# meta-pytorch/torchx

Measured on AMD Instinct MI355X. Metric: tokens_per_second, higher is better.
Workload: dtype bf16; 1 GPU; model=llama3_8b, global_batch=4, seq_len=4096, parallelism=dp1

## Files before the change

torchx_amd/models/llama.py:

```python

from __future__ import annotations

from dataclasses import dataclass
from typing import Optional

import torch
import torch.nn as nn

from torchx_amd import ops


@dataclass
class LlamaConfig:
    vocab_size: int = 128256
    hidden_size: int = 4096
    intermediate_size: int = 14336
    num_layers: int = 32
    num_heads: int = 32
    num_kv_heads: int = 8
    head_dim: int = 128
    max_seq_len: int = 8192
    rope_theta: float = 500000.0
    rms_eps: float = 1e-5
    tie_embeddings: bool = False

    @property
    def q_dim(self) -> int:
        return self.num_heads * self.head_dim

    @property
    def kv_dim(self) -> int:
        return self.num_kv_heads * self.head_dim


def llama3_8b() -> LlamaConfig:
    return LlamaConfig()

# ... 14 lines not shown
    )


def _lin(mod: nn.Module, x: torch.Tensor) -> torch.Tensor:
    if type(mod) is nn.Linear and mod.bias is None and x.is_cuda:
        return ops.fast_linear(x, mod.weight)
    return mod(x)


def _new_linear(in_features: int, out_features: int,
                device: Optional[torch.device]) -> nn.Linear:
    if device is not None and torch.device(device).type == "cuda":
        return torch.nn.utils.skip_init(
            nn.Linear, in_features, out_features, bias=False,
            dtype=torch.bfloat16, device=device)
    return nn.Linear(in_features, out_features, bias=False,
                     dtype=torch.bfloat16)


class LlamaBlock(nn.Module):
    def __init__(self, cfg: LlamaConfig,
                 device: Optional[torch.device] = None):
        super().__init__()
        self.cfg = cfg
        h, qd, kvd = cfg.hidden_size, cfg.q_dim, cfg.kv_dim
        self.wqkv = _new_linear(h, qd + 2 * kvd, device)
        self.wo = _new_linear(qd, h, device)
        self.wgu = _new_linear(h, 2 * cfg.intermediate_size, device)
        self.wdown = _new_linear(cfg.intermediate_size, h, device)
        self.attn_norm = nn.Parameter(torch.ones(h, dtype=torch.bfloat16))
        self.mlp_norm = nn.Parameter(torch.ones(h, dtype=torch.bfloat16))

    def forward(self, x: torch.Tensor, cos: torch.Tensor,
                sin: torch.Tensor) -> torch.Tensor:
        cfg = self.cfg
        B, S, H = x.shape
        xn = ops.rmsnorm(x, self.attn_norm, cfg.rms_eps)
        qkv = _lin(self.wqkv, xn)
        attn = ops.fused_attention_qkv(
            qkv, cos, sin, cfg.num_heads, cfg.num_kv_heads, causal=True
        )
        x = x + _lin(self.wo, attn.reshape(B, S, cfg.q_dim))
        xn = ops.rmsnorm(x, self.mlp_norm, cfg.rms_eps)
        x = x + _lin(self.wdown, ops.swiglu_packed(_lin(self.wgu, xn)))
        return x


class LlamaModel(nn.Module):

    def __init__(self, cfg: LlamaConfig, device: Optional[torch.device] = None):
        super().__init__()
        self.cfg = cfg
        factory = {"dtype": torch.bfloat16, "device": device}
        self.embed = nn.Embedding(cfg.vocab_size, cfg.hidden_size, **factory)
        self.blocks = nn.ModuleList(
            [LlamaBlock(cfg, device) for _ in range(cfg.num_layers)]
        )
        self.final_norm = nn.Parameter(
            torch.ones(cfg.hidden_size, dtype=torch.bfloat16)
        )
        self.lm_head = _new_linear(cfg.hidden_size, cfg.vocab_size, device)
        if cfg.tie_embeddings:
            self.lm_head.weight = self.embed.weight
        cos, sin = ops.rope_tables(cfg.max_seq_len, cfg.head_dim,
                                   cfg.rope_theta, device=device)
        self.register_buffer("rope_cos", cos, persistent=False)
        self.register_buffer("rope_sin", sin, persistent=False)
        if device is not None:
            self.to(device)
        self.apply(self._init_weights)

    def _init_weights(self, m: nn.Module) -> None:
        std = 0.02
        if isinstance(m, nn.Linear):
            nn.init.normal_(m.weight, mean=0.0, std=std)
        elif isinstance(m, nn.Embedding):
            nn.init.normal_(m.weight, mean=0.0, std=std)

    def forward_hidden(self, tokens: torch.Tensor) -> torch.Tensor:
        x = self.embed(tokens)
        cos, sin = self.rope_cos, self.rope_sin
        for blk in self.blocks:
            x = blk(x, cos, sin)
        return ops.rmsnorm(x, self.final_norm, self.cfg.rms_eps)

    def forward(self, tokens: torch.Tensor,
                targets: Optional[torch.Tensor] = None) -> torch.Tensor:
        x = self.forward_hidden(tokens)
        if targets is None:
            return self.lm_head(x)
        return ops.fused_linear_cross_entropy(
            x, self.lm_head.weight, targets
        )

    def num_params(self) -> int:
        return sum(p.numel() for p in self.parameters())
```

torchx_amd/ops/__init__.py:

```python

from __future__ import annotations

import importlib.util
import math
from pathlib import Path
from typing import Optional, Tuple

import torch

from . import reference

_SO = Path(__file__).resolve().parent / "_hip_ops.so"
_hip = None
_load_err: Optional[str] = None


def _load():
    global _hip, _load_err
    if _hip is not None:
        return _hip
    if not _SO.exists():
        _load_err = f"{_SO} not built (run torchx_amd/ops/build.py)"
        return None
    try:
# ... 15 lines not shown
            "back to eager."
        )
    return mod


def extension_available() -> bool:
    return _load() is not None


def _on_gpu(*ts: torch.Tensor) -> bool:
    return any(t.is_cuda for t in ts)




class _RMSNorm(torch.autograd.Function):
    @staticmethod
    def forward(ctx, x: torch.Tensor, w: torch.Tensor, eps: float):
        y, invrms = hip_ops().rmsnorm_fwd(x.contiguous(), w.contiguous(), eps)
        ctx.save_for_backward(x, w, invrms)
        return y

    @staticmethod
    def backward(ctx, dy: torch.Tensor):
        x, w, invrms = ctx.saved_tensors
        dx, dw = hip_ops().rmsnorm_bwd(dy.contiguous(), x, w, invrms)
        return dx, dw.to(w.dtype), None


def rmsnorm(x: torch.Tensor, w: torch.Tensor, eps: float = 1e-5) -> torch.Tensor:
    if _on_gpu(x):
        return _RMSNorm.apply(x, w, eps)
    return reference.rmsnorm(x, w, eps)




def rope_tables(
    seq_len: int, head_dim: int, theta: float = 500000.0,
    device: Optional[torch.device] = None,
) -> Tuple[torch.Tensor, torch.Tensor]:
    inv_freq = 1.0 / (
        theta ** (torch.arange(0, head_dim, 2, dtype=torch.float32) / head_dim)
    )
    pos = torch.arange(seq_len, dtype=torch.float32)
    ang = torch.outer(pos, inv_freq)
    cos, sin = torch.cos(ang), torch.sin(ang)
    if device is not None:
        cos, sin = cos.to(device), sin.to(device)
    return cos, sin


class _RoPE(torch.autograd.Function):
    @staticmethod
    def forward(ctx, x: torch.Tensor, cos: torch.Tensor, sin: torch.Tensor,
                heads: int):
        ctx.save_for_backward(cos, sin)
        ctx.heads = heads
        return hip_ops().rope(x.contiguous(), cos, sin, heads, 1.0)

    @staticmethod
    def backward(ctx, dy: torch.Tensor):
        cos, sin = ctx.saved_tensors
        dx = hip_ops().rope(dy.contiguous(), cos, sin, ctx.heads, -1.0)
        return dx, None, None, None

# ... 129 lines not shown
    def forward(ctx, q: torch.Tensor, k: torch.Tensor, v: torch.Tensor,
                causal: bool, scale: float):
        o, lse = hip_ops().attn_fwd(
            q.contiguous(), k.contiguous(), v.contiguous(), scale, causal
        )
        ctx.save_for_backward(q, k, v, o, lse)
        ctx.causal = causal
        ctx.scale = scale
        return o

    @staticmethod
    def backward(ctx, dout: torch.Tensor):
        q, k, v, o, lse = ctx.saved_tensors
        dq, dk, dv = hip_ops().attn_bwd(
            q, k, v, o, dout.contiguous(), lse, ctx.scale, ctx.causal
        )
        return dq, dk, dv, None, None


def set_attn_bwd_dq_mode(mode: str) -> None:
    hip_ops().set_attn_bwd_dq_mode(mode)


def get_attn_bwd_dq_mode() -> str:
    return hip_ops().get_attn_bwd_dq_mode()


def set_attn_bwd_dkv_impl(impl: str) -> None:
    hip_ops().set_attn_bwd_dkv_impl(impl)


def get_attn_bwd_dkv_impl() -> str:
    return hip_ops().get_attn_bwd_dkv_impl()


def flash_attention(
    q: torch.Tensor, k: torch.Tensor, v: torch.Tensor,
    causal: bool = True, scale: Optional[float] = None,
) -> torch.Tensor:
    if scale is None:
        scale = 1.0 / math.sqrt(q.shape[-1])
    if _on_gpu(q):
        return _FlashAttention.apply(q, k, v, causal, scale)
    return reference.attention(q, k, v, causal=causal, scale=scale)




def adamw_step(
    p32: torch.Tensor, p16: torch.Tensor, grad: torch.Tensor,
    m: torch.Tensor, v: torch.Tensor, *, lr: float, beta1: float = 0.9,
    beta2: float = 0.95, eps: float = 1e-8, weight_decay: float = 0.1,
    step: int = 1,
) -> None:
    if p32.is_cuda:
        hip_ops().adamw_step(p32, p16, grad, m, v, lr, beta1, beta2, eps,
                             weight_decay, step)
    else:
        reference.adamw_step(p32, p16, grad, m, v, lr=lr, beta1=beta1,
                             beta2=beta2, eps=eps, weight_decay=weight_decay,
                             step=step)


def mfma_probe(a: torch.Tensor, b: torch.Tensor) -> torch.Tensor:
    return hip_ops().mfma_probe(a, b)

# ... 347 lines not shown
```

torchx_amd/ops/csrc/attention.hip:

```cpp
#include "common.h"

#include <cstdlib>
#include <cstring>
#include <type_traits>

typedef __bf16 mbf16x8 __attribute__((ext_vector_type(8)));

#define HD 128
#define QBLK 32
#define KBLK 32
#define NWAVES 4
#define BLOCK_Q (QBLK * NWAVES)
#define BLOCK_K (KBLK * NWAVES)

__device__ __forceinline__ f32x16 mfma32(mbf16x8 a, mbf16x8 b, f32x16 c) {
  return __builtin_amdgcn_mfma_f32_32x32x16_bf16(a, b, c, 0, 0, 0);
}

__device__ __forceinline__ unsigned int pack_bf16x2(float a, float b) {
  unsigned int r;
  asm("v_cvt_pk_bf16_f32 %0, %1, %2" : "=v"(r) : "v"(a), "v"(b));
  return r;
}

// ... 115 lines not shown
  for (int p = 0; p < 4; ++p) {
    const int c = tid + p * 256;
    const int r = c >> 4, g = c & 15;
    #pragma unroll
    for (int j = 0; j < 8; ++j) {
      const int d = 8 * g + j;
      const int gr = ((r >> 3) + vrot(d)) & 7;
      *(unsigned short*)(vimg + d * 128 + gr * 16 + (r & 7) * 2) = vr[p][j];
    }
  }
}


__device__ __forceinline__ void map_block_fwd(int B, int Hq, int Hkv,
                                              int nqt, int G,
                                              int* b, int* hq, int* qt) {
  int bid = blockIdx.x;
  if (((B * Hkv) & 7) == 0) {
    const int gsz = G * nqt;
    const int xcd = bid & 7, slot = bid >> 3;
    const int g = (slot / gsz) * 8 + xcd;
    *b = g / Hkv;
    const int r = slot % gsz;
    *hq = (g % Hkv) * G + r / nqt;
    *qt = r % nqt;
  } else {
    *b = bid / (Hq * nqt);
    bid -= *b * Hq * nqt;
    *hq = bid / nqt;
    *qt = bid % nqt;
  }
}

template <int NTHREADS>
__device__ __forceinline__ void lds_nat_to_tr(const char* nat, char* tr_img) {
  const int tid = threadIdx.x;
  #pragma unroll
  for (int p = 0; p < 1024 / NTHREADS; ++p) {
    const int c = tid + p * NTHREADS;
    const int r = c >> 4, g = c & 15;
    const ushort8 v = *(const ushort8*)(
        nat + r * 256 + ((g * 16) ^ ((r & 15) << 4)));
    #pragma unroll
    for (int j = 0; j < 8; ++j) {
      const int d = 8 * g + j;
      const int gr = ((r >> 3) + vrot(d)) & 7;
      *(unsigned short*)(tr_img + d * 128 + gr * 16 + (r & 7) * 2) = v[j];
    }
  }
}



template <int NW = 4>
__device__ __forceinline__ void lds_nat_to_tr_own(const char* nat,
                                                  char* tr_img) {
  const int wave = threadIdx.x / 64;
  const int lane = threadIdx.x & 63;
  #pragma unroll
  for (int pp = 0; pp < 16 / NW; ++pp) {
    const int c = wave * (64 * 16 / NW) + pp * 64 + lane;
    const int r = c >> 4, g = c & 15;
    const ushort8 v = *(const ushort8*)(
        nat + r * 256 + ((g * 16) ^ ((r & 15) << 4)));
    #pragma unroll
    for (int j = 0; j < 8; ++j) {
      const int d = 8 * g + j;
      const int gr = ((r >> 3) + vrot(d)) & 7;
      *(unsigned short*)(tr_img + d * 128 + gr * 16 + (r & 7) * 2) = v[j];
    }
  }
}

template <int NW>
__global__ void __launch_bounds__(NW * 64, 2)
attn_fwd_kernel(const unsigned short* __restrict__ q,
                const unsigned short* __restrict__ k,
                const unsigned short* __restrict__ v,
                unsigned short* __restrict__ o,
                float* __restrict__ lse,
                int B, int S, int Hq, int Hkv, float scale, int causal,
                long q_rs, long kv_rs) {
  __shared__ __align__(16) char smem[4 * KIMG_BYTES];

  const int BQ = NW * QBLK;
  const int nqt = (S + BQ - 1) / BQ;
  const int G = Hq / Hkv;
  int b, hq, qt;
  map_block_fwd(B, Hq, Hkv, nqt, G, &b, &hq, &qt);
  const int hkv = hq / G;

  const int wave = threadIdx.x / 64;
  const int lane = threadIdx.x & 63;
  const bool hi = lane >= 32;
  const int qr = lane & 31;

  const long q_seq_stride = q_rs;
  const long kv_seq_stride = kv_rs;
  const unsigned short* qb = q + (long)b * S * q_seq_stride + (long)hq * HD;
  const unsigned short* kb = k + (long)b * S * kv_seq_stride + (long)hkv * HD;
  const unsigned short* vb = v + (long)b * S * kv_seq_stride + (long)hkv * HD;

  const int q0_blk = qt * BQ;
  const int qw0 = q0_blk + wave * QBLK;
  const long q_row = qw0 + qr;
  const bool wave_active = qw0 < S;

  mbf16x8 qfrag[8];
  {
    const long row = (q_row < S) ? q_row : (S - 1);
    const unsigned short* qp = qb + row * q_seq_stride + (hi ? 8 : 0);
    #pragma unroll
    for (int c = 0; c < 8; ++c) {
      qfrag[c] = __builtin_bit_cast(mbf16x8, *(const ushort8*)(qp + c * 16));
    }
  }

  f32x16 acc_o[4] = {};
  float m_run = -3.0e38f, l_run = 0.f;
  const float sc2 = scale * LOG2E;

  const int kv_limit = causal ? min(S, q0_blk + BQ) : S;
// ... 1318 lines not shown
    #pragma unroll
    for (int o = 0; o < 2; ++o) {
      unsigned short* out = o ? dk : dv;
      #pragma unroll
      for (int dt = 0; dt < 4; ++dt) {
        __syncthreads();
        #pragma unroll
        for (int r = 0; r < 16; ++r) {
          tr[c_row(r, hi) * 36 + kr] = o ? acck[dt][r] : accv[dt][r];
        }
        __syncthreads();
        #pragma unroll
        for (int rep = 0; rep < 4; ++rep) {
          const int kk = kr;
          const int d0 = (hi ? 16 : 0) + rep * 4;
          if (kw0 + kk < S) {
            bf16x4_raw w;
            #pragma unroll
            for (int j = 0; j < 4; ++j) {
              w[j] = (short)f32_to_bf16(tr[kk * 36 + d0 + j]);
            }
            *(bf16x4_raw*)(out + ((long)b * S + kw0 + kk) * out_rs +
                           (long)hkv * HD + dt * 32 + d0) = w;
          }
        }
      }
    }
  } else {
    #pragma unroll
    for (int i = 0; i < 16; ++i) __syncthreads();
  }
}

extern "C" void attn_fwd_launch(const void* q, const void* k, const void* v,
                                void* o, void* lse, int B, int S, int Hq,
                                int Hkv, float scale, int causal,
                                long q_rs, long kv_rs, hipStream_t stream) {
  static int fwd8 = -1;
  if (fwd8 < 0) {
    const char* e = getenv("TORCHX_AMD_FWD_8WAVE");
    fwd8 = (e && atoi(e)) ? 1 : 0;
  }
  if (fwd8 == 1) {
    const int nqt = (S + 8 * QBLK - 1) / (8 * QBLK);
    hipLaunchKernelGGL((attn_fwd_kernel<8>), dim3(B * Hq * nqt), dim3(512),
                       0, stream, (const unsigned short*)q,
                       (const unsigned short*)k, (const unsigned short*)v,
                       (unsigned short*)o, (float*)lse, B, S, Hq, Hkv,
                       scale, causal, q_rs, kv_rs);
  } else {
    const int nqt = (S + 4 * QBLK - 1) / (4 * QBLK);
    hipLaunchKernelGGL((attn_fwd_kernel<4>), dim3(B * Hq * nqt), dim3(256),
                       0, stream, (const unsigned short*)q,
                       (const unsigned short*)k, (const unsigned short*)v,
                       (unsigned short*)o, (float*)lse, B, S, Hq, Hkv,
                       scale, causal, q_rs, kv_rs);
  }
}

extern "C" void paged_prefill_attn_launch(
    const void* q, const void* kpool, const void* vpool, void* o,
    const void* bt, const void* ctx, int B, int S, int Hq, int Hkv,
    int num_pages, int logP, int M, float scale, hipStream_t stream) {
  const int nqt = (S + 4 * QBLK - 1) / (4 * QBLK);
  hipLaunchKernelGGL(paged_prefill_attn_kernel, dim3(B * Hq * nqt), dim3(256),
                     0, stream, (const unsigned short*)q,
                     (const unsigned short*)kpool,
                     (const unsigned short*)vpool, (unsigned short*)o,
                     (const int*)bt, (const int*)ctx, B, S, Hq, Hkv,
                     num_pages, logP, M, scale);
}

extern "C" void paged_prefill_attn_ragged_launch(
    const void* q, const void* kpool, const void* vpool, void* o,
    const void* bt, const void* ctx, const void* tiles, int ntiles, int B,
    int T, int Hq, int Hkv, int num_pages, int logP, int M, float scale,
    hipStream_t stream) {
  const long units = (long)ntiles * Hkv;
  const long grid = (units + 7) / 8 * 8 * (Hq / Hkv);
  hipLaunchKernelGGL(paged_prefill_attn_ragged_kernel, dim3((unsigned)grid),
                     dim3(256), 0, stream, (const unsigned short*)q,
                     (const unsigned short*)kpool,
                     (const unsigned short*)vpool, (unsigned short*)o,
                     (const int*)bt, (const int*)ctx, (const int4*)tiles,
                     ntiles, B, T, Hq, Hkv, num_pages, logP, M, scale);
}

static int g_dkv_merged = -1;

// ... 102 lines not shown
```

torchx_amd/ops/csrc/bindings.cpp:

```cpp
#include <torch/extension.h>
#include <c10/hip/HIPStream.h>

#include <hip/hip_runtime.h>

extern "C" {
void rope_launch(const void*, void*, const void*, const void*, long, int, int,
                 int, float, hipStream_t);
void swiglu_fwd_launch(const void*, const void*, void*, long, hipStream_t);
void swiglu_bwd_launch(const void*, const void*, const void*, void*, void*,
                       long, hipStream_t);
void rmsnorm_fwd_launch(const void*, const void*, void*, void*, long, int,
                        float, hipStream_t);
void rmsnorm_bwd_launch(const void*, const void*, const void*, const void*,
                        void*, void*, void*, long, int, hipStream_t);
long rmsnorm_bwd_dw_chunks(long);
void adamw_launch(void*, void*, const void*, void*, void*, long, float, float,
                  float, float, float, float, float, hipStream_t);
void ce_fwd_launch(const void*, const void*, void*, void*, long, int,
                   hipStream_t);
void ce_bwd_launch(const void*, const void*, const void*, const void*, void*,
                   long, int, hipStream_t);
void attn_fwd_launch(const void*, const void*, const void*, void*, void*, int,
                     int, int, int, float, int, long, long, hipStream_t);
void attn_bwd_launch(const void*, const void*, const void*, const void*,
                     const void*, const void*, void*, void*, void*, void*,
                     void*, int, int, int, int, float, int, long, long, long,
                     long, hipStream_t);
long attn_bwd_ds_bytes(int, int, int, int);
int attn_bwd_dkv_impl_get();
void attn_bwd_dkv_impl_set(int);
void rope_qkv_launch(const void*, void*, const void*, const void*, long, int,
                     long, int, float, hipStream_t);
void swiglu_gu_fwd_launch(const void*, void*, long, long, hipStream_t);
void swiglu_gu_bwd_launch(const void*, const void*, void*, long, long,
                          hipStream_t);
void mfma_probe_launch(const void*, const void*, void*, hipStream_t);
void mfma_probe_tr_launch(const void*, const void*, void*, void*,
                          hipStream_t);
void fp8_cast_transpose_launch(const void*, void*, void*, void*,
                               const void*, long, long, int, hipStream_t);
void transpose_bf16_launch(const void*, void*, long, long, hipStream_t);
void decode_attn_launch(const void*, const void*, const void*, void*,
                        const void*, int, int, int, int, int, int, float,
                        hipStream_t);
void gemv_bf16_launch(const void*, const void*, void*, int, int, int,
                      hipStream_t);
void decode_attn_split_launch(const void*, const void*, const void*, void*,
                              void*, void*, const void*, int, int, int, int,
                              int, int, int, float, hipStream_t);
void decode_rope_cache_launch(const void*, void*, void*, void*, const void*,
                              const void*, const void*, int, int, int, int,
                              int, int, hipStream_t);
void rmsnorm_res_launch(const void*, const void*, const void*, void*, void*,
                        long, int, float, hipStream_t);
void gemv_swiglu_launch(const void*, const void*, void*, int, int, int,
                        hipStream_t);
void paged_decode_attn_launch(const void*, const void*, const void*, void*,
                              void*, void*, const void*, const void*, int,
                              int, int, int, int, int, int, float,
                              hipStream_t);
void paged_decode_rope_cache_launch(const void*, void*, void*, void*,
                                    const void*, const void*, const void*,
                                    const void*, int, int, int, int, int,
                                    int, int, hipStream_t);
void paged_prefill_attn_launch(const void*, const void*, const void*, void*,
                               const void*, const void*, int, int, int, int,
                               int, int, int, float, hipStream_t);
void paged_prefill_attn_ragged_launch(const void*, const void*, const void*,
                                      void*, const void*, const void*,
                                      const void*, int, int, int, int, int,
                                      int, int, int, float, hipStream_t);
void paged_prefill_rope_cache_launch(const void*, void*, void*, void*,
                                     const void*, const void*, const void*,
                                     const void*, long, int, int, long, int,
                                     hipStream_t);
}

namespace {

hipStream_t cur_stream() {
  return c10::hip::getCurrentHIPStream().stream();
}

void check_bf16(const at::Tensor& t, const char* name) {
  TORCH_CHECK(t.is_cuda(), name, " must be on GPU");
  TORCH_CHECK(t.scalar_type() == at::kBFloat16, name, " must be bf16");
  TORCH_CHECK(t.is_contiguous(), name, " must be contiguous");
}

void check_f32(const at::Tensor& t, const char* name) {
  TORCH_CHECK(t.is_cuda(), name, " must be on GPU");
  TORCH_CHECK(t.scalar_type() == at::kFloat, name, " must be f32");
  TORCH_CHECK(t.is_contiguous(), name, " must be contiguous");
}

}

std::vector<at::Tensor> rmsnorm_fwd(at::Tensor x, at::Tensor w, double eps) {
  check_bf16(x, "x");
  check_bf16(w, "w");
  const long H = x.size(-1);
  TORCH_CHECK(H % 2048 == 0 && H <= 8192, "rmsnorm: H must be k*2048, <=8192");
  const long rows = x.numel() / H;
  auto y = at::empty_like(x);
  auto invrms = at::empty({rows}, x.options().dtype(at::kFloat));
  rmsnorm_fwd_launch(x.data_ptr(), w.data_ptr(), y.data_ptr(),
                     invrms.data_ptr(), rows, (int)H, (float)eps,
                     cur_stream());
  return {y, invrms};
}

std::vector<at::Tensor> rmsnorm_bwd(at::Tensor dy, at::Tensor x, at::Tensor w,
                                    at::Tensor invrms) {
  check_bf16(dy, "dy");
  check_bf16(x, "x");
  const long H = x.size(-1);
  TORCH_CHECK(H % 2048 == 0 && H <= 8192, "rmsnorm: H must be k*2048, <=8192");
  const long rows = x.numel() / H;
  auto dx = at::empty_like(x);
  auto dw = at::empty({H}, x.options().dtype(at::kFloat));
  auto dw_part = at::empty({rmsnorm_bwd_dw_chunks(rows), H}, dw.options());
  rmsnorm_bwd_launch(dy.data_ptr(), x.data_ptr(), w.data_ptr(),
                     invrms.data_ptr(), dx.data_ptr(), dw.data_ptr(),
                     dw_part.data_ptr(), rows, (int)H, cur_stream());
  return {dx, dw};
}

at::Tensor rope(at::Tensor x, at::Tensor cos_t, at::Tensor sin_t, long heads,
                double sign) {
  check_bf16(x, "x");
  check_f32(cos_t, "cos");
  check_f32(sin_t, "sin");
  const long D = x.size(-1);
  const long rows = x.numel() / D;
  const long S = cos_t.size(0);
  TORCH_CHECK(cos_t.size(1) == D / 2, "cos table must be [S, D/2]");
  auto y = at::empty_like(x);
  rope_launch(x.data_ptr(), y.data_ptr(), cos_t.data_ptr(), sin_t.data_ptr(),
              rows, (int)D, (int)heads, (int)S, (float)sign, cur_stream());
  return y;
}

at::Tensor swiglu_fwd(at::Tensor g, at::Tensor u) {
  check_bf16(g, "g");
  check_bf16(u, "u");
  auto out = at::empty_like(g);
  swiglu_fwd_launch(g.data_ptr(), u.data_ptr(), out.data_ptr(), g.numel(),
                    cur_stream());
  return out;
}

std::vector<at::Tensor> swiglu_bwd(at::Tensor dout, at::Tensor g,
                                   at::Tensor u) {
  check_bf16(dout, "dout");
  auto dg = at::empty_like(g);
  auto du = at::empty_like(u);
// ... 60 lines not shown
  return {o, lse};
}

int g_dq_stream = -1;

bool dq_stream_mode() {
  if (g_dq_stream < 0) {
    const char* e = getenv("TORCHX_AMD_DQ_MODE");
    g_dq_stream = (e && std::string(e) == "recompute") ? 0 : 1;
  }
  return g_dq_stream == 1;
}

void set_attn_bwd_dq_mode(const std::string& mode) {
  TORCH_CHECK(mode == "stream" || mode == "recompute",
              "attn bwd dq mode must be 'stream' or 'recompute', got '",
              mode, "'");
  g_dq_stream = (mode == "stream") ? 1 : 0;
}

std::string get_attn_bwd_dq_mode() {
  return dq_stream_mode() ? "stream" : "recompute";
}

void set_attn_bwd_dkv_impl(const std::string& impl) {
  TORCH_CHECK(impl == "merged" || impl == "split",
              "attn bwd dkv impl must be 'merged' or 'split', got '", impl,
              "'");
  attn_bwd_dkv_impl_set(impl == "merged" ? 1 : 0);
}

std::string get_attn_bwd_dkv_impl() {
  return attn_bwd_dkv_impl_get() == 1 ? "merged" : "split";
}

constexpr long kDsScratchCapBytes = 8L << 30;

at::Tensor alloc_ds_scratch(const at::Tensor& like, int B, int S, int Hq,
                            bool causal) {
  if (!dq_stream_mode()) return at::Tensor();
  const long bytes = attn_bwd_ds_bytes(B, S, Hq, causal ? 1 : 0);
  if (bytes > kDsScratchCapBytes) return at::Tensor();
  return at::empty({bytes}, like.options().dtype(at::kByte));
}

std::vector<at::Tensor> attn_bwd(at::Tensor q, at::Tensor k, at::Tensor v,
                                 at::Tensor o, at::Tensor dout, at::Tensor lse,
                                 double scale, bool causal) {
  check_bf16(dout, "dout");
  const int B = q.size(0), S = q.size(1), Hq = q.size(2);
  const int Hkv = k.size(2);
  auto dq = at::empty_like(q);
  auto dk = at::empty_like(k);
  auto dv = at::empty_like(v);
  auto delta = at::empty({B, Hq, S}, q.options().dtype(at::kFloat));
  auto ds = alloc_ds_scratch(q, B, S, Hq, causal);
  attn_bwd_launch(q.data_ptr(), k.data_ptr(), v.data_ptr(), o.data_ptr(),
                  dout.data_ptr(), lse.data_ptr(), delta.data_ptr(),
                  dq.data_ptr(), dk.data_ptr(), dv.data_ptr(),
                  ds.defined() ? ds.data_ptr() : nullptr, B, S, Hq, Hkv,
                  (float)scale, causal ? 1 : 0, (long)Hq * 128,
                  (long)Hkv * 128, (long)Hq * 128, (long)Hkv * 128,
                  cur_stream());
  return {dq, dk, dv};
}

// ... 394 lines not shown
              "cos/sin must be [S, 64] (head_dim 128)");
  const long nh = qkv.size(1) / 128;
  const int Hq = (int)nh - 2 * Hkv;
  TORCH_CHECK(Hq >= 1 && qkv.size(1) == nh * 128, "qkv width mismatch");
  TORCH_CHECK(Hq % Hkv == 0, "GQA group mismatch");
  const int rope_rows = (int)std::min<long>(cos_t.size(0), 1L << 30);
  auto q = at::empty({T, (long)Hq, 128}, qkv.options());
  paged_prefill_rope_cache_launch(
      qkv.data_ptr(), q.data_ptr(), kpool.data_ptr(), vpool.data_ptr(),
      cos_t.data_ptr(), sin_t.data_ptr(), pos.data_ptr(), slot.data_ptr(), T,
      Hq, Hkv, pool_rows, rope_rows, cur_stream());
  return q;
}

std::vector<at::Tensor> rmsnorm_res(at::Tensor x,
                                    c10::optional<at::Tensor> res,
                                    at::Tensor w, double eps) {
  check_bf16(x, "x");
  check_bf16(w, "w");
  const long H = x.size(-1);
  TORCH_CHECK(H % 2048 == 0 && H <= 8192, "rmsnorm: H must be k*2048, <=8192");
  const long R = x.numel() / H;
  auto y = at::empty_like(x);
  at::Tensor s = x;
  const void* rp = nullptr;
  void* sp = nullptr;
  if (res.has_value()) {
    check_bf16(*res, "res");
    TORCH_CHECK(res->sizes() == x.sizes(), "res shape mismatch");
    s = at::empty_like(x);
    rp = res->data_ptr();
    sp = s.data_ptr();
  }
  rmsnorm_res_launch(x.data_ptr(), rp, w.data_ptr(), sp, y.data_ptr(), R,
                     (int)H, (float)eps, cur_stream());
  return {s, y};
}

std::vector<at::Tensor> mfma_probe_tr(at::Tensor a, at::Tensor b) {
  check_bf16(a, "a");
  check_bf16(b, "b");
  TORCH_CHECK(a.size(0) == 32 && a.size(1) == 16, "a must be [32,16]");
  TORCH_CHECK(b.size(0) == 16 && b.size(1) == 32, "b must be [16,32]");
  auto c = at::empty({32, 32}, a.options().dtype(at::kFloat));
  auto raw = at::empty({64, 8}, a.options());
  mfma_probe_tr_launch(a.data_ptr(), b.data_ptr(), c.data_ptr(),
                       raw.data_ptr(), cur_stream());
  return {c, raw};
}

at::Tensor mfma_probe(at::Tensor a, at::Tensor b) {
  check_bf16(a, "a");
  check_bf16(b, "b");
  TORCH_CHECK(a.size(0) == 32 && a.size(1) == 16, "a must be [32,16]");
  TORCH_CHECK(b.size(0) == 16 && b.size(1) == 32, "b must be [16,32]");
  auto c = at::empty({32, 32}, a.options().dtype(at::kFloat));
  mfma_probe_launch(a.data_ptr(), b.data_ptr(), c.data_ptr(), cur_stream());
  return c;
}

PYBIND11_MODULE(TORCH_EXTENSION_NAME, m) {
  m.def("rmsnorm_fwd", &rmsnorm_fwd);
  m.def("rmsnorm_bwd", &rmsnorm_bwd);
  m.def("rope", &rope);
  m.def("swiglu_fwd", &swiglu_fwd);
  m.def("swiglu_bwd", &swiglu_bwd);
  m.def("adamw_step", &adamw_step);
  m.def("ce_fwd", &ce_fwd);
  m.def("ce_bwd", &ce_bwd);
  m.def("attn_fwd", &attn_fwd);
  m.def("attn_bwd", &attn_bwd);
  m.def("set_attn_bwd_dq_mode", &set_attn_bwd_dq_mode);
  m.def("get_attn_bwd_dq_mode", &get_attn_bwd_dq_mode);
  m.def("set_attn_bwd_dkv_impl", &set_attn_bwd_dkv_impl);
  m.def("get_attn_bwd_dkv_impl", &get_attn_bwd_dkv_impl);
  m.def("attn_fwd_qkv", &attn_fwd_qkv);
  m.def("attn_bwd_qkv", &attn_bwd_qkv);
  m.def("rope_qkv", &rope_qkv);
  m.def("swiglu_gu_fwd", &swiglu_gu_fwd);
  m.def("swiglu_gu_bwd", &swiglu_gu_bwd);
  m.def("fp8_cast_transpose", &fp8_cast_transpose);
  m.def("mfma_probe", &mfma_probe);
  m.def("mfma_probe_tr", &mfma_probe_tr);
  m.def("transpose_bf16", &transpose_bf16);
  m.def("decode_attn", &decode_attn);
  m.def("decode_attn_dev", &decode_attn_dev);
  m.def("gemv_bf16", &gemv_bf16);
  m.def("gemv_swiglu_bf16", &gemv_swiglu_bf16);
  m.def("decode_rope_cache", &decode_rope_cache,
        py::arg("qkv"), py::arg("kc"), py::arg("vc"), py::arg("cos"),
        py::arg("sin"), py::arg("pos") = 0,
        py::arg("pos_dev") = c10::nullopt);
  m.def("paged_decode_attn", &paged_decode_attn);
  m.def("paged_decode_rope_cache", &paged_decode_rope_cache);
  m.def("paged_prefill_attn", &paged_prefill_attn);
  m.def("paged_prefill_attn_ragged", &paged_prefill_attn_ragged);
  m.def("paged_prefill_rope_cache", &paged_prefill_rope_cache);
  m.def("rmsnorm_res", &rmsnorm_res,
        py::arg("x"), py::arg("res"), py::arg("w"), py::arg("eps"));
}
```

torchx_amd/ops/csrc/rmsnorm.hip:

```cpp
#include "common.h"

template <int ITERS>
__global__ void __launch_bounds__(256)
rmsnorm_fwd_kernel(
    const unsigned short* __restrict__ x,
    const unsigned short* __restrict__ w,
    unsigned short* __restrict__ y,
    float* __restrict__ invrms,
    int H, float eps) {
  __shared__ float red[4];
  const long row = blockIdx.x;
  const unsigned short* xr = x + row * (long)H;
  unsigned short* yr = y + row * (long)H;

  float xs[ITERS][8];
  float acc = 0.f;
  #pragma unroll
  for (int it = 0; it < ITERS; ++it) {
    int i = (it * 256 + threadIdx.x) * 8;
    ushort8 v = *(const ushort8*)(xr + i);
    #pragma unroll
    for (int j = 0; j < 8; ++j) {
      float f = bf16_to_f32(v[j]);
      xs[it][j] = f;
      acc = fmaf(f, f, acc);
    }
  }
  float total = block_reduce<4>(acc, red,
      [] __device__ (float a, float b) { return a + b; });
  float r = rsqrtf(total / (float)H + eps);
  if (threadIdx.x == 0) invrms[row] = r;

  #pragma unroll
  for (int it = 0; it < ITERS; ++it) {
    int i = (it * 256 + threadIdx.x) * 8;
    ushort8 wv = *(const ushort8*)(w + i);
    ushort8 ov;
    #pragma unroll
    for (int j = 0; j < 8; ++j) {
      ov[j] = f32_to_bf16(xs[it][j] * r * bf16_to_f32(wv[j]));
    }
    *(ushort8*)(yr + i) = ov;
  }
}


template <int ITERS>
__global__ void __launch_bounds__(256)
rmsnorm_bwd_dx_kernel(
    const unsigned short* __restrict__ dy,
    const unsigned short* __restrict__ x,
    const unsigned short* __restrict__ w,
    const float* __restrict__ invrms,
    unsigned short* __restrict__ dx,
    int H) {
  __shared__ float red[4];
  const long row = blockIdx.x;
  const unsigned short* xr = x + row * (long)H;
  const unsigned short* dyr = dy + row * (long)H;
  unsigned short* dxr = dx + row * (long)H;
  const float r = invrms[row];

  float xs[ITERS][8], dyw[ITERS][8];
  float t = 0.f;
  #pragma unroll
  for (int it = 0; it < ITERS; ++it) {
    int i = (it * 256 + threadIdx.x) * 8;
    ushort8 xv = *(const ushort8*)(xr + i);
    ushort8 dv = *(const ushort8*)(dyr + i);
    ushort8 wv = *(const ushort8*)(w + i);
    #pragma unroll
    for (int j = 0; j < 8; ++j) {
      float xf = bf16_to_f32(xv[j]);
      float dwf = bf16_to_f32(dv[j]) * bf16_to_f32(wv[j]);
      xs[it][j] = xf;
      dyw[it][j] = dwf;
      t = fmaf(dwf, xf, t);
    }
  }
  float ts = block_reduce<4>(t, red,
      [] __device__ (float a, float b) { return a + b; });
  const float kk = ts * r * r * r / (float)H;

  #pragma unroll
  for (int it = 0; it < ITERS; ++it) {
    int i = (it * 256 + threadIdx.x) * 8;
    ushort8 ov;
    #pragma unroll
    for (int j = 0; j < 8; ++j) {
      ov[j] = f32_to_bf16(fmaf(dyw[it][j], r, -xs[it][j] * kk));
    }
    *(ushort8*)(dxr + i) = ov;
  }
}

#define DW_CHUNK_ROWS 64

__global__ void __launch_bounds__(256)
rmsnorm_bwd_dw_kernel(
    const unsigned short* __restrict__ dy,
    const unsigned short* __restrict__ x,
    const float* __restrict__ invrms,
    float* __restrict__ part,
    long rows, int H) {
  const int col = (blockIdx.y * 2048) + threadIdx.x * 8;
  const long row0 = (long)blockIdx.x * DW_CHUNK_ROWS;
  const long row1 = min(row0 + DW_CHUNK_ROWS, rows);
  float acc[8] = {0.f, 0.f, 0.f, 0.f, 0.f, 0.f, 0.f, 0.f};
  for (long row = row0; row < row1; ++row) {
    const float r = invrms[row];
    ushort8 xv = *(const ushort8*)(x + row * (long)H + col);
    ushort8 dv = *(const ushort8*)(dy + row * (long)H + col);
    #pragma unroll
    for (int j = 0; j < 8; ++j) {
      acc[j] = fmaf(bf16_to_f32(dv[j]) * bf16_to_f32(xv[j]), r, acc[j]);
    }
  }
  float* out = part + (long)blockIdx.x * H + col;
  #pragma unroll
  for (int j = 0; j < 8; ++j) out[j] = acc[j];
}

__global__ void __launch_bounds__(256)
// ... 10 lines not shown
  red[group][lane] = s;
  __syncthreads();
  if (group == 0) {
    dw[col] = (red[0][lane] + red[1][lane]) + (red[2][lane] + red[3][lane]);
  }
}

extern "C" long rmsnorm_bwd_dw_chunks(long rows) {
  return (rows + DW_CHUNK_ROWS - 1) / DW_CHUNK_ROWS;
}

#define DISPATCH_ITERS(H, FN)                                                  \
  do {                                                                         \
    int iters = (H) / 2048;                                                    \
    if (iters == 1) FN(1);                                                     \
    else if (iters == 2) FN(2);                                                \
    else if (iters == 3) FN(3);                                                \
    else if (iters == 4) FN(4);                                                \
  } while (0)

extern "C" void rmsnorm_fwd_launch(const void* x, const void* w, void* y,
                                   void* invrms, long rows, int H, float eps,
                                   hipStream_t stream) {
#define LAUNCH_F(I)                                                            \
  hipLaunchKernelGGL((rmsnorm_fwd_kernel<I>), dim3((int)rows), dim3(256), 0,   \
                     stream, (const unsigned short*)x,                         \
                     (const unsigned short*)w, (unsigned short*)y,             \
                     (float*)invrms, H, eps)
  DISPATCH_ITERS(H, LAUNCH_F);
#undef LAUNCH_F
}

extern "C" void rmsnorm_bwd_launch(const void* dy, const void* x,
                                   const void* w, const void* invrms, void* dx,
                                   void* dw, void* dw_part, long rows, int H,
                                   hipStream_t stream) {
#define LAUNCH_B(I)                                                            \
  hipLaunchKernelGGL((rmsnorm_bwd_dx_kernel<I>), dim3((int)rows), dim3(256),   \
                     0, stream, (const unsigned short*)dy,                     \
                     (const unsigned short*)x, (const unsigned short*)w,       \
                     (const float*)invrms, (unsigned short*)dx, H)
  DISPATCH_ITERS(H, LAUNCH_B);
#undef LAUNCH_B
  const int row_chunks = (int)rmsnorm_bwd_dw_chunks(rows);
  if (row_chunks > 0) {
    hipLaunchKernelGGL(rmsnorm_bwd_dw_kernel,
                       dim3(row_chunks, H / 2048), dim3(256), 0, stream,
                       (const unsigned short*)dy, (const unsigned short*)x,
                       (const float*)invrms, (float*)dw_part, rows, H);
  }
  hipLaunchKernelGGL(rmsnorm_bwd_dw_reduce_kernel, dim3(H / 64), dim3(256), 0,
                     stream, (const float*)dw_part, (float*)dw, row_chunks, H);
}

template <int ITERS>
__global__ void __launch_bounds__(256)
rmsnorm_res_fwd_kernel(const unsigned short* __restrict__ x,
                       const unsigned short* __restrict__ res,
                       const unsigned short* __restrict__ w,
                       unsigned short* __restrict__ s_out,
                       unsigned short* __restrict__ y,
                       int H, float eps) {
  __shared__ float red[4];
  const long row = blockIdx.x;
  const unsigned short* xr = x + row * (long)H;
  unsigned short* yr = y + row * (long)H;

  float xs[ITERS][8];
  float acc = 0.f;
  #pragma unroll
  for (int it = 0; it < ITERS; ++it) {
    int i = (it * 256 + threadIdx.x) * 8;
    ushort8 v = *(const ushort8*)(xr + i);
    ushort8 rv;
    if (res) rv = *(const ushort8*)(res + row * (long)H + i);
    ushort8 sv;
    #pragma unroll
    for (int j = 0; j < 8; ++j) {
      float f = bf16_to_f32(v[j]);
      if (res) {
        f += bf16_to_f32(rv[j]);
        sv[j] = f32_to_bf16(f);
        f = bf16_to_f32(sv[j]);
      }
      xs[it][j] = f;
      acc = fmaf(f, f, acc);
    }
    if (res) *(ushort8*)(s_out + row * (long)H + i) = sv;
  }
  float total = block_reduce<4>(acc, red,
      [] __device__ (float a, float b) { return a + b; });
  float r = rsqrtf(total / (float)H + eps);

  #pragma unroll
  for (int it = 0; it < ITERS; ++it) {
    int i = (it * 256 + threadIdx.x) * 8;
    ushort8 wv = *(const ushort8*)(w + i);
    ushort8 ov;
    #pragma unroll
    for (int j = 0; j < 8; ++j) {
      ov[j] = f32_to_bf16(xs[it][j] * r * bf16_to_f32(wv[j]));
    }
    *(ushort8*)(yr + i) = ov;
  }
}

extern "C" void rmsnorm_res_launch(const void* x, const void* res,
                                   const void* w, void* s_out, void* y,
                                   long R, int H, float eps,
                                   hipStream_t stream) {
  #define RMSRES_CASE(N)                                                   \
    case N:                                                                \
      hipLaunchKernelGGL((rmsnorm_res_fwd_kernel<N>), dim3(R), dim3(256),  \
                         0, stream, (const unsigned short*)x,              \
                         (const unsigned short*)res,                       \
                         (const unsigned short*)w, (unsigned short*)s_out, \
                         (unsigned short*)y, H, eps);                      \
      break;
  switch (H / 2048) {
    RMSRES_CASE(1)
    RMSRES_CASE(2)
    RMSRES_CASE(3)
    RMSRES_CASE(4)
    default: break;
  }
  #undef RMSRES_CASE
}
```

Before: 21660 tokens/s.

## Fuse residual add into RMSNorm and add balanced XCD-aware attention forward mapping

Each block now returns the residual and the MLP output separately, so the next block's residual add is fused into its attention RMSNorm through a new add_rmsnorm kernel. The backward pass folds the residual gradient into the rmsnorm dx kernel. Together these remove separate elementwise add kernels and their memory traffic in both passes. Separately, the attention forward kernel gets a new default 'balanced' block mapping that spreads KV streams across the 8 XCDs and schedules heavy causal tiles first, with padding and early exit when the stream count is not a multiple of 8.

```diff
diff --git a/torchx_amd/models/llama.py b/torchx_amd/models/llama.py
--- a/torchx_amd/models/llama.py
+++ b/torchx_amd/models/llama.py
@@ -2,7 +2,7 @@
 from __future__ import annotations
 
 from dataclasses import dataclass
-from typing import Optional
+from typing import Optional, Tuple
 
 import torch
 import torch.nn as nn
@@ -83,18 +83,22 @@
         self.mlp_norm = nn.Parameter(torch.ones(h, dtype=torch.bfloat16))
 
     def forward(self, x: torch.Tensor, cos: torch.Tensor,
-                sin: torch.Tensor) -> torch.Tensor:
+                sin: torch.Tensor, delta: Optional[torch.Tensor] = None
+                ) -> Tuple[torch.Tensor, torch.Tensor]:
         cfg = self.cfg
         B, S, H = x.shape
-        xn = ops.rmsnorm(x, self.attn_norm, cfg.rms_eps)
+        if delta is None:
+            xn = ops.rmsnorm(x, self.attn_norm, cfg.rms_eps)
+        else:
+            x, xn = ops.add_rmsnorm(x, delta, self.attn_norm, cfg.rms_eps)
         qkv = _lin(self.wqkv, xn)
         attn = ops.fused_attention_qkv(
             qkv, cos, sin, cfg.num_heads, cfg.num_kv_heads, causal=True
         )
-        x = x + _lin(self.wo, attn.reshape(B, S, cfg.q_dim))
-        xn = ops.rmsnorm(x, self.mlp_norm, cfg.rms_eps)
-        x = x + _lin(self.wdown, ops.swiglu_packed(_lin(self.wgu, xn)))
-        return x
+        x, xn = ops.add_rmsnorm(
+            x, _lin(self.wo, attn.reshape(B, S, cfg.q_dim)), self.mlp_norm,
+            cfg.rms_eps)
+        return x, _lin(self.wdown, ops.swiglu_packed(_lin(self.wgu, xn)))
 
 
 class LlamaModel(nn.Module):
@@ -131,9 +135,13 @@
     def forward_hidden(self, tokens: torch.Tensor) -> torch.Tensor:
         x = self.embed(tokens)
         cos, sin = self.rope_cos, self.rope_sin
+        delta = None
         for blk in self.blocks:
-            x = blk(x, cos, sin)
-        return ops.rmsnorm(x, self.final_norm, self.cfg.rms_eps)
+            x, delta = blk(x, cos, sin, delta)
+        if delta is None:
+            return ops.rmsnorm(x, self.final_norm, self.cfg.rms_eps)
+        return ops.add_rmsnorm(x, delta, self.final_norm,
+                               self.cfg.rms_eps)[1]
 
     def forward(self, tokens: torch.Tensor,
                 targets: Optional[torch.Tensor] = None) -> torch.Tensor:
diff --git a/torchx_amd/ops/__init__.py b/torchx_amd/ops/__init__.py
--- a/torchx_amd/ops/__init__.py
+++ b/torchx_amd/ops/__init__.py
@@ -71,6 +71,36 @@
     if _on_gpu(x):
         return _RMSNorm.apply(x, w, eps)
     return reference.rmsnorm(x, w, eps)
+
+
+class _AddRMSNorm(torch.autograd.Function):
+    @staticmethod
+    def forward(ctx, x: torch.Tensor, delta: torch.Tensor, w: torch.Tensor,
+                eps: float):
+        s, y, invrms = hip_ops().add_rmsnorm_fwd(
+            x.contiguous(), delta.contiguous(), w.contiguous(), eps)
+        ctx.save_for_backward(s, w, invrms)
+        ctx.set_materialize_grads(False)
+        return s, y
+
+    @staticmethod
+    def backward(ctx, ds: Optional[torch.Tensor],
+                 dy: Optional[torch.Tensor]):
+        if dy is None:
+            return ds, ds, None, None
+        s, w, invrms = ctx.saved_tensors
+        dx, dw = hip_ops().rmsnorm_bwd(
+            dy.contiguous(), s, w, invrms,
+            ds.contiguous() if ds is not None else None)
+        return dx, dx, dw.to(w.dtype), None
+
+
+def add_rmsnorm(x: torch.Tensor, delta: torch.Tensor, w: torch.Tensor,
+                eps: float = 1e-5) -> Tuple[torch.Tensor, torch.Tensor]:
+    if _on_gpu(x):
+        return _AddRMSNorm.apply(x, delta, w, eps)
+    s = x + delta
+    return s, reference.rmsnorm(s, w, eps)
 
 
 
@@ -266,6 +296,14 @@
 
 def get_attn_bwd_dkv_impl() -> str:
     return hip_ops().get_attn_bwd_dkv_impl()
+
+
+def set_attn_fwd_map(name: str) -> None:
+    hip_ops().set_attn_fwd_map(name)
+
+
+def get_attn_fwd_map() -> str:
+    return hip_ops().get_attn_fwd_map()
 
 
 def flash_attention(
diff --git a/torchx_amd/ops/csrc/attention.hip b/torchx_amd/ops/csrc/attention.hip
--- a/torchx_amd/ops/csrc/attention.hip
+++ b/torchx_amd/ops/csrc/attention.hip
@@ -171,6 +171,30 @@
   }
 }
 
+__device__ __forceinline__ bool map_block_fwd_balanced(int B, int Hq, int Hkv,
+                                                       int nqt, int G,
+                                                       int heavy, int* b,
+                                                       int* hq, int* qt) {
+  const int xcd = blockIdx.x & 7, slot = blockIdx.x >> 3;
+  const int u = slot / G;
+  const int nstream = B * Hkv;
+  int g, t;
+  if ((nstream & 7) == 0) {
+    const int ns = nstream >> 3;
+    g = (u % ns) * 8 + xcd;
+    t = u / ns;
+  } else {
+    const int unit = u * 8 + xcd;
+    if (unit >= nstream * nqt) return false;
+    g = unit % nstream;
+    t = unit / nstream;
+  }
+  *b = g / Hkv;
+  *hq = (g % Hkv) * G + slot % G;
+  *qt = heavy ? nqt - 1 - t : t;
+  return true;
+}
+
 template <int NTHREADS>
 __device__ __forceinline__ void lds_nat_to_tr(const char* nat, char* tr_img) {
   const int tid = threadIdx.x;
@@ -219,14 +243,20 @@
                 unsigned short* __restrict__ o,
                 float* __restrict__ lse,
                 int B, int S, int Hq, int Hkv, float scale, int causal,
-                long q_rs, long kv_rs) {
+                long q_rs, long kv_rs,
+                int map) {
   __shared__ __align__(16) char smem[4 * KIMG_BYTES];
 
   const int BQ = NW * QBLK;
   const int nqt = (S + BQ - 1) / BQ;
   const int G = Hq / Hkv;
   int b, hq, qt;
-  map_block_fwd(B, Hq, Hkv, nqt, G, &b, &hq, &qt);
+  if (map == 0) {
+    map_block_fwd(B, Hq, Hkv, nqt, G, &b, &hq, &qt);
+  } else if (!map_block_fwd_balanced(B, Hq, Hkv, nqt, G, map == 1, &b, &hq,
+                                     &qt)) {
+    return;
+  }
   const int hkv = hq / G;
 
   const int wave = threadIdx.x / 64;
@@ -1611,6 +1641,24 @@
   }
 }
 
+#define ATTN_FWD_MAP_DEFAULT 1
+static int g_fwd_map = -1;
+
+extern "C" int attn_fwd_map_get() {
+  if (g_fwd_map < 0) {
+    const char* e = getenv("TORCHX_AMD_FWD_MAP");
+    g_fwd_map = !e ? ATTN_FWD_MAP_DEFAULT
+              : strcmp(e, "legacy") == 0 ? 0
+              : strcmp(e, "balanced") == 0 ? 1
+              : strcmp(e, "adjacent") == 0 ? 2 : ATTN_FWD_MAP_DEFAULT;
+  }
+  return g_fwd_map;
+}
+
+extern "C" void attn_fwd_map_set(int map) {
+  g_fwd_map = (map >= 0 && map <= 2) ? map : ATTN_FWD_MAP_DEFAULT;
+}
+
 extern "C" void attn_fwd_launch(const void* q, const void* k, const void* v,
                                 void* o, void* lse, int B, int S, int Hq,
                                 int Hkv, float scale, int causal,
@@ -1626,14 +1674,19 @@
                        0, stream, (const unsigned short*)q,
                        (const unsigned short*)k, (const unsigned short*)v,
                        (unsigned short*)o, (float*)lse, B, S, Hq, Hkv,
-                       scale, causal, q_rs, kv_rs);
+                       scale, causal, q_rs, kv_rs, 0);
   } else {
     const int nqt = (S + 4 * QBLK - 1) / (4 * QBLK);
-    hipLaunchKernelGGL((attn_fwd_kernel<4>), dim3(B * Hq * nqt), dim3(256),
+    const int map = attn_fwd_map_get();
+    long grid = (long)B * Hq * nqt;
+    if (map != 0 && ((B * Hkv) & 7) != 0) {
+      grid = ((long)B * Hkv * nqt + 7) / 8 * 8 * (Hq / Hkv);
+    }
+    hipLaunchKernelGGL((attn_fwd_kernel<4>), dim3((unsigned)grid), dim3(256),
                        0, stream, (const unsigned short*)q,
                        (const unsigned short*)k, (const unsigned short*)v,
                        (unsigned short*)o, (float*)lse, B, S, Hq, Hkv,
-                       scale, causal, q_rs, kv_rs);
+                       scale, causal, q_rs, kv_rs, map);
   }
 }
 
diff --git a/torchx_amd/ops/csrc/bindings.cpp b/torchx_amd/ops/csrc/bindings.cpp
--- a/torchx_amd/ops/csrc/bindings.cpp
+++ b/torchx_amd/ops/csrc/bindings.cpp
@@ -12,7 +12,8 @@
 void rmsnorm_fwd_launch(const void*, const void*, void*, void*, long, int,
                         float, hipStream_t);
 void rmsnorm_bwd_launch(const void*, const void*, const void*, const void*,
-                        void*, void*, void*, long, int, hipStream_t);
+                        const void*, void*, void*, void*, long, int,
+                        hipStream_t);
 long rmsnorm_bwd_dw_chunks(long);
 void adamw_launch(void*, void*, const void*, void*, void*, long, float, float,
                   float, float, float, float, float, hipStream_t);
@@ -29,6 +30,8 @@
 long attn_bwd_ds_bytes(int, int, int, int);
 int attn_bwd_dkv_impl_get();
 void attn_bwd_dkv_impl_set(int);
+int attn_fwd_map_get();
+void attn_fwd_map_set(int);
 void rope_qkv_launch(const void*, void*, const void*, const void*, long, int,
                      long, int, float, hipStream_t);
 void swiglu_gu_fwd_launch(const void*, void*, long, long, hipStream_t);
@@ -52,7 +55,7 @@
                               const void*, const void*, int, int, int, int,
                               int, int, hipStream_t);
 void rmsnorm_res_launch(const void*, const void*, const void*, void*, void*,
-                        long, int, float, hipStream_t);
+                        void*, long, int, float, hipStream_t);
 void gemv_swiglu_launch(const void*, const void*, void*, int, int, int,
                         hipStream_t);
 void paged_decode_attn_launch(const void*, const void*, const void*, void*,
@@ -111,17 +114,29 @@
 }
 
 std::vector<at::Tensor> rmsnorm_bwd(at::Tensor dy, at::Tensor x, at::Tensor w,
-                                    at::Tensor invrms) {
+                                    at::Tensor invrms,
+                                    c10::optional<at::Tensor> dres) {
   check_bf16(dy, "dy");
   check_bf16(x, "x");
+  check_bf16(w, "w");
+  check_f32(invrms, "invrms");
   const long H = x.size(-1);
   TORCH_CHECK(H % 2048 == 0 && H <= 8192, "rmsnorm: H must be k*2048, <=8192");
   const long rows = x.numel() / H;
+  TORCH_CHECK(dy.sizes() == x.sizes(), "dy shape mismatch");
+  TORCH_CHECK(w.numel() == H && invrms.numel() == rows,
+              "w / invrms size mismatch");
+  const void* rp = nullptr;
+  if (dres.has_value()) {
+    check_bf16(*dres, "dres");
+    TORCH_CHECK(dres->sizes() == x.sizes(), "dres shape mismatch");
+    rp = dres->data_ptr();
+  }
   auto dx = at::empty_like(x);
   auto dw = at::empty({H}, x.options().dtype(at::kFloat));
   auto dw_part = at::empty({rmsnorm_bwd_dw_chunks(rows), H}, dw.options());
   rmsnorm_bwd_launch(dy.data_ptr(), x.data_ptr(), w.data_ptr(),
-                     invrms.data_ptr(), dx.data_ptr(), dw.data_ptr(),
+                     invrms.data_ptr(), rp, dx.data_ptr(), dw.data_ptr(),
                      dw_part.data_ptr(), rows, (int)H, cur_stream());
   return {dx, dw};
 }
@@ -248,6 +263,18 @@
 
 std::string get_attn_bwd_dkv_impl() {
   return attn_bwd_dkv_impl_get() == 1 ? "merged" : "split";
+}
+
+void set_attn_fwd_map(const std::string& name) {
+  TORCH_CHECK(name == "legacy" || name == "balanced" || name == "adjacent",
+              "attn fwd map must be 'balanced', 'legacy' or 'adjacent', "
+              "got '", name, "'");
+  attn_fwd_map_set(name == "legacy" ? 0 : name == "balanced" ? 1 : 2);
+}
+
+std::string get_attn_fwd_map() {
+  const int m = attn_fwd_map_get();
+  return m == 0 ? "legacy" : m == 1 ? "balanced" : "adjacent";
 }
 
 constexpr long kDsScratchCapBytes = 8L << 30;
@@ -708,9 +735,28 @@
     rp = res->data_ptr();
     sp = s.data_ptr();
   }
-  rmsnorm_res_launch(x.data_ptr(), rp, w.data_ptr(), sp, y.data_ptr(), R,
-                     (int)H, (float)eps, cur_stream());
+  rmsnorm_res_launch(x.data_ptr(), rp, w.data_ptr(), sp, y.data_ptr(),
+                     nullptr, R, (int)H, (float)eps, cur_stream());
   return {s, y};
+}
+
+std::vector<at::Tensor> add_rmsnorm_fwd(at::Tensor x, at::Tensor delta,
+                                        at::Tensor w, double eps) {
+  check_bf16(x, "x");
+  check_bf16(delta, "delta");
+  check_bf16(w, "w");
+  const long H = x.size(-1);
+  TORCH_CHECK(H % 2048 == 0 && H <= 8192, "rmsnorm: H must be k*2048, <=8192");
+  TORCH_CHECK(delta.sizes() == x.sizes(), "delta shape mismatch");
+  TORCH_CHECK(w.numel() == H, "w size mismatch");
+  const long R = x.numel() / H;
+  auto s = at::empty_like(x);
+  auto y = at::empty_like(x);
+  auto invrms = at::empty({R}, x.options().dtype(at::kFloat));
+  rmsnorm_res_launch(x.data_ptr(), delta.data_ptr(), w.data_ptr(),
+                     s.data_ptr(), y.data_ptr(), invrms.data_ptr(), R, (int)H,
+                     (float)eps, cur_stream());
+  return {s, y, invrms};
 }
 
 std::vector<at::Tensor> mfma_probe_tr(at::Tensor a, at::Tensor b) {
@@ -737,7 +783,9 @@
 
 PYBIND11_MODULE(TORCH_EXTENSION_NAME, m) {
   m.def("rmsnorm_fwd", &rmsnorm_fwd);
-  m.def("rmsnorm_bwd", &rmsnorm_bwd);
+  m.def("rmsnorm_bwd", &rmsnorm_bwd, py::arg("dy"), py::arg("x"),
+        py::arg("w"), py::arg("invrms"), py::arg("dres") = c10::nullopt);
+  m.def("add_rmsnorm_fwd", &add_rmsnorm_fwd);
   m.def("rope", &rope);
   m.def("swiglu_fwd", &swiglu_fwd);
   m.def("swiglu_bwd", &swiglu_bwd);
@@ -750,6 +798,8 @@
   m.def("get_attn_bwd_dq_mode", &get_attn_bwd_dq_mode);
   m.def("set_attn_bwd_dkv_impl", &set_attn_bwd_dkv_impl);
   m.def("get_attn_bwd_dkv_impl", &get_attn_bwd_dkv_impl);
+  m.def("set_attn_fwd_map", &set_attn_fwd_map);
+  m.def("get_attn_fwd_map", &get_attn_fwd_map);
   m.def("attn_fwd_qkv", &attn_fwd_qkv);
   m.def("attn_bwd_qkv", &attn_bwd_qkv);
   m.def("rope_qkv", &rope_qkv);
diff --git a/torchx_amd/ops/csrc/rmsnorm.hip b/torchx_amd/ops/csrc/rmsnorm.hip
--- a/torchx_amd/ops/csrc/rmsnorm.hip
+++ b/torchx_amd/ops/csrc/rmsnorm.hip
@@ -52,6 +52,7 @@
     const unsigned short* __restrict__ x,
     const unsigned short* __restrict__ w,
     const float* __restrict__ invrms,
+    const unsigned short* __restrict__ dres,
     unsigned short* __restrict__ dx,
     int H) {
   __shared__ float red[4];
@@ -89,6 +90,13 @@
     #pragma unroll
     for (int j = 0; j < 8; ++j) {
       ov[j] = f32_to_bf16(fmaf(dyw[it][j], r, -xs[it][j] * kk));
+    }
+    if (dres) {
+      ushort8 rv = *(const ushort8*)(dres + row * (long)H + i);
+      #pragma unroll
+      for (int j = 0; j < 8; ++j) {
+        ov[j] = f32_to_bf16(bf16_to_f32(ov[j]) + bf16_to_f32(rv[j]));
+      }
     }
     *(ushort8*)(dxr + i) = ov;
   }
@@ -165,14 +173,16 @@
 }
 
 extern "C" void rmsnorm_bwd_launch(const void* dy, const void* x,
-                                   const void* w, const void* invrms, void* dx,
-                                   void* dw, void* dw_part, long rows, int H,
+                                   const void* w, const void* invrms,
+                                   const void* dres, void* dx, void* dw,
+                                   void* dw_part, long rows, int H,
                                    hipStream_t stream) {
 #define LAUNCH_B(I)                                                            \
   hipLaunchKernelGGL((rmsnorm_bwd_dx_kernel<I>), dim3((int)rows), dim3(256),   \
                      0, stream, (const unsigned short*)dy,                     \
                      (const unsigned short*)x, (const unsigned short*)w,       \
-                     (const float*)invrms, (unsigned short*)dx, H)
+                     (const float*)invrms, (const unsigned short*)dres,      \
+                     (unsigned short*)dx, H)
   DISPATCH_ITERS(H, LAUNCH_B);
 #undef LAUNCH_B
   const int row_chunks = (int)rmsnorm_bwd_dw_chunks(rows);
@@ -193,6 +203,7 @@
                        const unsigned short* __restrict__ w,
                        unsigned short* __restrict__ s_out,
                        unsigned short* __restrict__ y,
+                       float* __restrict__ invrms,
                        int H, float eps) {
   __shared__ float red[4];
   const long row = blockIdx.x;
@@ -224,6 +235,7 @@
   float total = block_reduce<4>(acc, red,
       [] __device__ (float a, float b) { return a + b; });
   float r = rsqrtf(total / (float)H + eps);
+  if (invrms && threadIdx.x == 0) invrms[row] = r;
 
   #pragma unroll
   for (int it = 0; it < ITERS; ++it) {
@@ -240,7 +252,7 @@
 
 extern "C" void rmsnorm_res_launch(const void* x, const void* res,
                                    const void* w, void* s_out, void* y,
-                                   long R, int H, float eps,
+                                   void* invrms, long R, int H, float eps,
                                    hipStream_t stream) {
   #define RMSRES_CASE(N)                                                   \
     case N:                                                                \
@@ -248,7 +260,7 @@
                          0, stream, (const unsigned short*)x,              \
                          (const unsigned short*)res,                       \
                          (const unsigned short*)w, (unsigned short*)s_out, \
-                         (unsigned short*)y, H, eps);                      \
+                         (unsigned short*)y, (float*)invrms, H, eps);      \
       break;
   switch (H / 2048) {
     RMSRES_CASE(1)
```

Result: faster. 21890 tokens/s (median of 6 runs) (+1.1%).
